# thygate/stable-diffusion-webui-depthmap-script

Measured on AMD Instinct MI355X. Metric: depth+stereo pairs/sec @1024x1024, higher is better.
Workload: dtype f16 (network) / f64 (stereo, normal map); 1 GPU; BASELINE config c3: MiDaS 3.1 DPT BEiT-L/16 512 forward (fp16, random-init weights seed 0, net 512x512, 1025 tokens) + depth->u16 + create_stereoimages(polylines_sharp, left-right, divergence 2.5%) + create_normalmap (Sobel 3) on 32 x 1024x1024 RGB per GPU, inputs resident in HBM; depth_network=dpt_beit_large_512, height=1024, width=1024, forward_launch=eager, library_convolutions=MIOpen, heuristic solver choice, overlap=single stream, parallelism=units sharded over 1 GPU(s), no data-path collective

## Files before the change

stable-diffusion-webui-depthmap-script_amd/csrc/ds_linear.hip:

```cpp
#include "ds_common.h"

#include <stdlib.h>
#include <atomic>
#include <type_traits>

typedef _Float16 lf16x8 __attribute__((ext_vector_type(8)));
typedef __bf16 lbf16x8 __attribute__((ext_vector_type(8)));
typedef _Float16 lf16x4 __attribute__((ext_vector_type(4)));
typedef __bf16 lbf16x4 __attribute__((ext_vector_type(4)));
typedef float lf32x16 __attribute__((ext_vector_type(16)));
typedef float lf32x4 __attribute__((ext_vector_type(4)));

#if defined(DS_EXPERIMENTS) && defined(DS_LIN_MFMA32)
#define LN_MF16 0
#else
#define LN_MF16 1
#endif

#define LN_THREADS 512
#define LN_LDS_BYTES 131072
#define LN_HALF 16384
#define LN_B_BASE 65536

template <int BF16> struct ln_traits;
template <> struct ln_traits<0> {
    typedef _Float16 T; typedef lf16x8 V8; typedef lf16x4 V4;
    static __device__ __forceinline__ lf32x16 mfma(V8 a, V8 b, lf32x16 c) { return __builtin_amdgcn_mfma_f32_32x32x16_f16(a, b, c, 0, 0, 0); }
    static __device__ __forceinline__ lf32x4 mfma16(V8 a, V8 b, lf32x4 c) { return __builtin_amdgcn_mfma_f32_16x16x32_f16(a, b, c, 0, 0, 0); }
    static __device__ __forceinline__ V8 relu(V8 v)
    {
        typedef unsigned lu32x4 __attribute__((ext_vector_type(4)));
        const lu32x4 x = __builtin_bit_cast(lu32x4, v);
        unsigned r0, r1, r2, r3;
        asm("v_pk_max_f16 %0, %1, 0" : "=v"(r0) : "v"(x[0]));
        asm("v_pk_max_f16 %0, %1, 0" : "=v"(r1) : "v"(x[1]));
        asm("v_pk_max_f16 %0, %1, 0" : "=v"(r2) : "v"(x[2]));
        asm("v_pk_max_f16 %0, %1, 0" : "=v"(r3) : "v"(x[3]));
        return __builtin_bit_cast(V8, (lu32x4){r0, r1, r2, r3});
    }
};
template <> struct ln_traits<1> {
    typedef __bf16 T; typedef lbf16x8 V8; typedef lbf16x4 V4;
    static __device__ __forceinline__ lf32x16 mfma(V8 a, V8 b, lf32x16 c) { return __builtin_amdgcn_mfma_f32_32x32x16_bf16(a, b, c, 0, 0, 0); }
    static __device__ __forceinline__ lf32x4 mfma16(V8 a, V8 b, lf32x4 c) { return __builtin_amdgcn_mfma_f32_16x16x32_bf16(a, b, c, 0, 0, 0); }
    static __device__ __forceinline__ V8 relu(V8 v)
    {
        typedef unsigned lu32x4 __attribute__((ext_vector_type(4)));
        lu32x4 x = __builtin_bit_cast(lu32x4, v);
#pragma unroll
        for (int i = 0; i < 4; ++i) {
            const unsigned neg = (x[i] >> 15) & 0x00010001u;
            x[i] &= ~(neg * 0xffffu);
        }
        return __builtin_bit_cast(V8, x);
    }
};

struct LinParams {
    const void *x, *w, *bias;
    const void *res1, *res2;
    const void *zeros;
    void *y;
    int M, N, K;
    int nbm, nbn;
    int bnw;
    int ablate;
    int stagger;
    int H, W, C, cpt, magic;
    long long ldy;
    const void *gamma;
    int early;
    int n_main;
    int vt_np, vt_c;
    unsigned vt_magic;
    int ps_w, ps_s, ps_c;
    unsigned ps_w_magic, ps_c_magic;
    int rd_np, rd_n, rd_dummy;
    unsigned rd_magic;
    float *rg_ws;
    int *rg_cnt;
    int rg_ksl;
    int th_nrb;
    int kt_kind;
    const float2 *ln_stats;
    const float *ln_colsum;
};

__device__ __forceinline__ void ln_tile_origin(const LinParams &P, const int tile, int &bm0, int &bn0)
{
    const int grp8 = tile / (8 * P.nbn), rem8 = tile - grp8 * (8 * P.nbn);
    const int rows8 = min(8, P.nbm - 8 * grp8);
    const int bn = rem8 / rows8, bm = 8 * grp8 + (rem8 - bn * rows8);
    bm0 = min(bm * 256, P.M - 256);
    bn0 = bn * P.bnw;
}

template <int VT>
__device__ __forceinline__ size_t ln_out_off(const LinParams &P, const int row, const int col)
{
    if (VT == 0) return (size_t)row * P.ldy + col;
    if (VT == 1) {
        const unsigned b = __umulhi((unsigned)col, P.vt_magic);
        const unsigned n = (unsigned)col - b * (unsigned)P.vt_np;
        return ((size_t)b * P.vt_c + row) * (size_t)P.vt_np + n;
    }
    if (VT == 2) {
        const unsigned q = __umulhi((unsigned)row, P.ps_w_magic), x = (unsigned)row - q * (unsigned)P.ps_w;
        const unsigned t = __umulhi((unsigned)col, P.ps_c_magic), co = (unsigned)col - t * (unsigned)P.ps_c;
        const unsigned ky = t / (unsigned)P.ps_s, kx = t - ky * (unsigned)P.ps_s;
        const size_t opix = ((size_t)q * P.ps_s + ky) * ((size_t)P.ps_w * P.ps_s) + (size_t)x * P.ps_s + kx;
        return opix * (size_t)P.ps_c + co;
    }
    const unsigned b = __umulhi((unsigned)row, P.rd_magic), t = (unsigned)row - b * (unsigned)P.rd_np;
    const bool live = t >= 1u && t < (unsigned)P.rd_n;
    const size_t orow = live ? (size_t)b * (size_t)(P.rd_n - 1) + (t - 1u) : (size_t)P.rd_dummy;
    return orow * (size_t)P.ldy + col;
}
template <int VT>
__device__ __forceinline__ size_t ln_res_off(const LinParams &P, const int row, const int col)
{
    if (VT != 3) return ln_out_off<VT>(P, row, col);
    const unsigned b = __umulhi((unsigned)row, P.rd_magic);
    return (size_t)b * (size_t)P.ldy + col;
}

__device__ __forceinline__ float ln_gelu(float v)
{
    const float u = fminf(fabsf(v), 6.0f);
    float q = 1.8896206483987044e-06f;
    q = __builtin_fmaf(q, u, -6.268127617659047e-05f);
    q = __builtin_fmaf(q, u, 0.000938866869546473f);
    q = __builtin_fmaf(q, u, -0.008539456874132156f);
    q = __builtin_fmaf(q, u, 0.054020676761865616f);
    q = __builtin_fmaf(q, u, 0.45840978622436523f);
    q = __builtin_fmaf(q, u, 1.1512691974639893f);
    q = __builtin_fmaf(q, u, 0.9999943375587463f);
    const float h = __builtin_amdgcn_exp2f(-q);
    return __builtin_fmaf(-u, h, fmaxf(v, 0.0f));
}
typedef float lf32x2 __attribute__((ext_vector_type(2)));
__device__ __forceinline__ lf32x2 ln_gelu2(lf32x2 v)
{
    const lf32x2 u = {fminf(fabsf(v[0]), 6.0f), fminf(fabsf(v[1]), 6.0f)};
    lf32x2 q = {1.8896206483987044e-06f, 1.8896206483987044e-06f};
#define LN_PK(c) q = __builtin_elementwise_fma(q, u, (lf32x2){c, c})
    LN_PK(-6.268127617659047e-05f); LN_PK(0.000938866869546473f); LN_PK(-0.008539456874132156f); LN_PK(0.054020676761865616f);
    LN_PK(0.45840978622436523f); LN_PK(1.1512691974639893f); LN_PK(0.9999943375587463f);
#undef LN_PK
    const lf32x2 h = {__builtin_amdgcn_exp2f(-q[0]), __builtin_amdgcn_exp2f(-q[1])};
    const lf32x2 r = {fmaxf(v[0], 0.0f), fmaxf(v[1], 0.0f)};
    return __builtin_elementwise_fma(-u, h, r);
}

__device__ __forceinline__ void ln_dma_s(const void *base_uniform, unsigned voff, unsigned lds_uniform)
{
    asm volatile("s_mov_b32 m0, %2\n\ts_nop 0\n\tglobal_load_lds_dwordx4 %0, %1" ::"v"(voff), "s"(base_uniform), "s"(lds_uniform) : "memory");
}
__device__ __forceinline__ void ln_dma_v(const void *ptr, unsigned lds_uniform)
{
    asm volatile("s_mov_b32 m0, %1\n\ts_nop 0\n\tglobal_load_lds_dwordx4 %0, off" ::"v"(ptr), "s"(lds_uniform) : "memory");
}

#ifdef DS_EXPERIMENTS
#define LN_ABLATE(bit) (P.ablate & (bit))
#define LN_STAGGER() (P.stagger)
#else
#define LN_ABLATE(bit) 0
#define LN_STAGGER() 0
#endif
#define LN_WAIT_VM(n) asm volatile("s_waitcnt vmcnt(" #n ")" ::: "memory")
template <int N> __device__ __forceinline__ void ln_wait_vm() { asm volatile("s_waitcnt vmcnt(%0)" ::"n"(N) : "memory"); }
#define LN_WAIT_LGKM0() asm volatile("s_waitcnt lgkmcnt(0)" ::: "memory")
#define LN_BARRIER()                              \
    do {                                          \
        __builtin_amdgcn_sched_barrier(0);        \
        __builtin_amdgcn_s_barrier();             \
        __builtin_amdgcn_sched_barrier(0);        \
    } while (0)

template <int BF16, int EPI, int CONV, int RES, int VT = 0, int NH = 0>
__global__ __launch_bounds__(LN_THREADS) void k_linear256(LinParams P)
{
    typedef ln_traits<BF16> TR;
    typedef typename TR::T T;
    typedef typename TR::V8 V8;
    extern __shared__ __attribute__((aligned(1024))) unsigned char lds[];

    const int tid = threadIdx.x;
    const int lane = tid & 63;
    const int wid = __builtin_amdgcn_readfirstlane(tid >> 6);
    const int wr = wid >> 2, wc = wid & 3;

    const int nwg = P.n_main;
    const int K = P.K;
    const int rowbytes = (CONV ? P.C : K) * (int)sizeof(T);

    unsigned srcA[2], srcB[2];
    int rowA[2];
#pragma unroll
    for (int i = 0; i < 2; ++i) {
        const int c = 2 * wid + i;
        const int j = 8 * c + (lane >> 3);
        const int slot = (lane & 7) ^ ((j >> 1) & 7);
        rowA[i] = (j >> 6) * 128 + (j & 63);
        srcA[i] = (unsigned)rowA[i] * (unsigned)rowbytes + slot * 16;
        const int col = NH ? j : (j >> 5) * 64 + (j & 31);
        srcB[i] = (unsigned)col * (unsigned)K * (unsigned)sizeof(T) + slot * 16;
    }
    const unsigned a_half = 64u * (unsigned)rowbytes;
    const unsigned b_half = NH ? 0u : 32u * (unsigned)K * (unsigned)sizeof(T);
    const unsigned lds_stage = (unsigned)(size_t)(__attribute__((address_space(3))) void *)lds + (unsigned)(2 * wid) * 1024u;

    int bm0 = 0, bn0 = 0;
    const unsigned char *xb = nullptr, *wb = nullptr;
    unsigned okA = 0;
    auto set_tile = [&](const int orig) {
        const int xcd = orig & 7, q8 = nwg >> 3, r8 = nwg & 7;
        const int tile = (xcd < r8 ? xcd * (q8 + 1) : r8 * (q8 + 1) + (xcd - r8) * q8) + (orig >> 3);
        ln_tile_origin(P, tile, bm0, bn0);
        xb = (const unsigned char *)P.x + (size_t)bm0 * rowbytes;
        wb = (const unsigned char *)P.w + (size_t)bn0 * K * sizeof(T);
        if (CONV) {
            okA = 0;
#pragma unroll
            for (int i = 0; i < 2; ++i)
#pragma unroll
                for (int h = 0; h < 2; ++h) {
                    const unsigned pix = (unsigned)(bm0 + rowA[i] + 64 * h) % (unsigned)(P.H * P.W);
                    const int py = (int)(pix / (unsigned)P.W), px = (int)(pix % (unsigned)P.W);
                    const unsigned bits = (py > 0 ? 1u : 0u) | 2u | (py < P.H - 1 ? 4u : 0u) | (px > 0 ? 8u : 0u) | 16u | (px < P.W - 1 ? 32u : 0u);
                    okA |= bits << (6 * (2 * h + i));
                }
        }
    };

#define LN_STAGE(kind, kt, s)                                                                                            \
    do {                                                                                                                 \
        unsigned koff_ = (unsigned)(kt) * 128u;                                                                          \
        const unsigned dst_ = ((kind) >> 1) * LN_B_BASE + ((kind) & 1) * 2 * LN_HALF + (s) * LN_HALF + lds_stage;   \
        int dy_ = 0, dx_ = 0, aoff_ = (int)koff_;                                                                        \
        if (CONV) {               \
            const int cc_ = ((kt) * 7282) >> 16, tap_ = (kt) - 9 * cc_;       \
            dy_ = ((tap_ * 11) >> 5) - 1; dx_ = tap_ - 3 * (dy_ + 1) - 1;                                                \
            aoff_ = cc_ * 128 + (dy_ * P.W + dx_) * rowbytes;                                                            \
            koff_ = (unsigned)(tap_ * P.cpt + cc_) * 128u;                            \
        }                                                                                                                \
                   \
        const unsigned char *ub_ = ((kind) < 2) ? xb + ((long)aoff_ + (long)(((kind) & 1) * a_half))                     \
                                                : wb + (size_t)(((kind) & 1) * b_half + koff_);                          \
        _Pragma("unroll") for (int i_ = 0; i_ < 2; ++i_) {                                                               \
            if (CONV && (kind) < 2) {                                                                                    \
                const unsigned sh_ = 6 * (2 * ((kind) & 1) + i_);                                                        \
                const unsigned ok_ = (okA >> (sh_ + dy_ + 1)) & (okA >> (sh_ + 4 + dx_)) & 1u;                           \
                const unsigned char *g_ = ok_ ? ub_ + (size_t)srcA[i_] : (const unsigned char *)P.zeros;                 \
                ln_dma_v(g_, dst_ + i_ * 1024);                                                                          \
            } else {                                                                                                     \
                ln_dma_s(ub_, ((kind) < 2) ? srcA[i_] : srcB[i_], dst_ + i_ * 1024);                                     \
            }                                                                                                            \
        }                                                                                                                \
    } while (0)

    constexpr bool MF16 = LN_MF16 && CONV == 0;
    constexpr int NKS = MF16 ? 2 : 4;
    unsigned offA[NKS], offB[NKS];
#pragma unroll
    for (int ks = 0; ks < NKS; ++ks) {
        const int lrow = MF16 ? (lane & 15) : (lane & 31);
        const unsigned sl = (unsigned)((MF16 ? 4 * ks + (lane >> 4) : 2 * ks + (lane >> 5)) ^ ((lane >> 1) & 7)) << 4;
        offA[ks] = (unsigned)(wr * 64 + lrow) * 128u + sl;
        offB[ks] = LN_B_BASE + (unsigned)(wc * 32 + lrow) * 128u + sl;
    }
    const int c8 = MF16 ? 16 * ((lane >> 4) & 1) + 8 * (lane >> 5) : 8 * (lane >> 5);
    constexpr int NBK = MF16 ? 1 : 2;
    constexpr int NBIAS = 2 * NBK;
    V8 bv[2][2];
#define LN_LOAD_BIAS()                                                                                                   \
    do {                                                                                                                 \
        const T *bias_ = (const T *)P.bias;                                                                              \
        _Pragma("unroll") for (int hb_ = 0; hb_ < 2; ++hb_) _Pragma("unroll") for (int k_ = 0; k_ < NBK; ++k_) {         \
            const int c_ = bn0 + (NH ? wc * 32 : wc * 64 + hb_ * 32) + c8 + 16 * k_;                                     \
            bv[hb_][k_] = *(const V8 *)(bias_ ? bias_ + c_ : (const T *)P.w);                                            \
        }                                                                                                                \
    } while (0)
#define LN_ZERO_NULL_BIAS()                                                                                              \
    do {                                                                                                                 \
        if (!P.bias) {                                                                                                   \
            _Pragma("unroll") for (int hb_ = 0; hb_ < 2; ++hb_) _Pragma("unroll") for (int k_ = 0; k_ < NBK; ++k_)       \
                _Pragma("unroll") for (int t_ = 0; t_ < 8; ++t_) bv[hb_][k_][t_] = (T)0.f;                               \
        }                                                                                                                \
    } while (0)
    V8 fa[2][2][4];
    V8 fb[2][4];
    lf32x16 acc[2][2][2];
    V8 fa16[2][4][2];
    V8 fb16[2][2][2];
    lf32x4 acc16[2][4][2][2];

#define LN_READ_A(h, s)                                                                                                  \
    do {                                                                                                                 \
        if constexpr (MF16) {                                                                                            \
            _Pragma("unroll") for (int rb_ = 0; rb_ < 4; ++rb_) _Pragma("unroll") for (int ks_ = 0; ks_ < 2; ++ks_)      \
                fa16[h][rb_][ks_] = *(const V8 *)(lds + offA[ks_] + ((h) * 2 * LN_HALF + (s) * LN_HALF + rb_ * 2048));   \
        } else {                                                                                                         \
            _Pragma("unroll") for (int rb_ = 0; rb_ < 2; ++rb_) _Pragma("unroll") for (int ks_ = 0; ks_ < 4; ++ks_)      \
                fa[h][rb_][ks_] = *(const V8 *)(lds + offA[ks_] + ((h) * 2 * LN_HALF + (s) * LN_HALF + rb_ * 4096));     \
        }                                                                                                                \
    } while (0)
#define LN_RELU_A(h)                                                                                                     \
    do {                                                                                                                 \
        if constexpr (CONV == 2) {                                                                                       \
            _Pragma("unroll") for (int rb_ = 0; rb_ < 2; ++rb_) _Pragma("unroll") for (int ks_ = 0; ks_ < 4; ++ks_)      \
                fa[h][rb_][ks_] = TR::relu(fa[h][rb_][ks_]);                                                             \
        }                                                                                                                \
    } while (0)
#define LN_READ_B(h, s)                                                                                                  \
    do {                                                                                                                 \
        if constexpr (MF16) {                                                                                            \
            _Pragma("unroll") for (int cb_ = 0; cb_ < 2; ++cb_) _Pragma("unroll") for (int ks_ = 0; ks_ < 2; ++ks_)      \
                if (!(NH && (h) == 1)) fb16[h][cb_][ks_] = *(const V8 *)(lds + offB[ks_] + ((h) * 2 * LN_HALF + (s) * LN_HALF + cb_ * 2048)); \
        } else {                                                                                                         \
            _Pragma("unroll") for (int ks_ = 0; ks_ < 4; ++ks_)                                                          \
                if (!(NH && (h) == 1)) fb[h][ks_] = *(const V8 *)(lds + offB[ks_] + ((h) * 2 * LN_HALF + (s) * LN_HALF)); \
        }                                                                                                                \
    } while (0)
#define LN_MMA_PART(ha, hb)                                                                                              \
    do {                                                                                                                 \
        if (!(NH && (hb) == 1)) {                                                                                        \
            if constexpr (MF16) {                                                                                        \
                _Pragma("unroll") for (int ks_ = 0; ks_ < 2; ++ks_) _Pragma("unroll") for (int rb_ = 0; rb_ < 4; ++rb_)  \
                    _Pragma("unroll") for (int cb_ = 0; cb_ < 2; ++cb_)                                                  \
                        acc16[ha][rb_][hb][cb_] = TR::mfma16(fb16[hb][cb_][ks_], fa16[ha][rb_][ks_], acc16[ha][rb_][hb][cb_]); \
            } else {                                                                                                     \
                _Pragma("unroll") for (int ks_ = 0; ks_ < 4; ++ks_) _Pragma("unroll") for (int rb_ = 0; rb_ < 2; ++rb_)  \
                    acc[ha][rb_][hb] = TR::mfma(fb[hb][ks_], fa[ha][rb_][ks_], acc[ha][rb_][hb]);                        \
            }                                                                                                            \
        }                                                                                                                \
    } while (0)

    const int nt = K >> 6, ni = nt >> 1;

#define LN_PROLOGUE()                                                                                                    \
    do {                                                                                                                 \
        LN_STAGE(0, 0, 0); LN_STAGE(2, 0, 0); LN_STAGE(3, 0, 0); LN_STAGE(1, 0, 0);                                      \
        LN_STAGE(0, 1, 1); LN_STAGE(2, 1, 1); LN_STAGE(3, 1, 1);                                                         \
    } while (0)

#define LN_PHASE_END(ha, hb)                                                                                             \
    do {                                                                                                                 \
        LN_BARRIER(); LN_WAIT_LGKM0();                                                                                   \
        __builtin_amdgcn_s_setprio(1);                                                                                   \
        LN_MMA_PART(ha, hb);                                                                                             \
        __builtin_amdgcn_s_setprio(0);                                                                                   \
        LN_BARRIER();                                                                                                    \
    } while (0)
#define LN_MEM(READ, STAGE)                                                                                              \
    do { READ; STAGE; } while (0)

    auto iteration = [&](const int i, auto kind_c) {
        constexpr int KIND = decltype(kind_c)::value;
        constexpr bool LAST = KIND == 1;
        const int e2 = 2 * i + 2, o2 = 2 * i + 3;
#define LN_WAIT_HEAD()                                                                                                   \
        do {                                                                                                             \
            if constexpr (KIND == 2) { if constexpr (NH) LN_WAIT_VM(18); else LN_WAIT_VM(26); }                          \
            else if constexpr (KIND == 1) ln_wait_vm<10 + NBIAS>();                                                   \
            else LN_WAIT_VM(10);                                                                                         \
        } while (0)
        LN_MEM(LN_READ_B(0, 0), LN_STAGE(1, 2 * i + 1, 1)); LN_WAIT_HEAD();
        LN_PHASE_END(0, 0);
        if constexpr (!LAST) { LN_MEM(LN_READ_B(1, 0), LN_STAGE(0, e2, 0)); LN_WAIT_HEAD(); } else { LN_READ_B(1, 0); ln_wait_vm<8 + NBIAS>(); }
        LN_PHASE_END(0, 1);
        if constexpr (!LAST) { LN_MEM(LN_READ_A(1, 0), LN_STAGE(2, e2, 0)); LN_RELU_A(1); LN_WAIT_HEAD(); } else { LN_READ_A(1, 0); LN_RELU_A(1); ln_wait_vm<6 + NBIAS>(); }
        LN_PHASE_END(1, 1);
        if constexpr (!LAST) { LN_MEM(LN_READ_A(0, 1), LN_STAGE(3, e2, 0)); LN_RELU_A(0); LN_WAIT_HEAD(); } else { LN_READ_A(0, 1); LN_RELU_A(0); ln_wait_vm<4 + NBIAS>(); }
        LN_PHASE_END(1, 0);
        if constexpr (!LAST) { LN_MEM(LN_READ_B(0, 1), LN_STAGE(1, e2, 0)); LN_WAIT_HEAD(); } else { LN_READ_B(0, 1); ln_wait_vm<2 + NBIAS>(); }
        LN_PHASE_END(0, 0);
#undef LN_WAIT_HEAD
        if constexpr (!LAST) { LN_MEM(LN_READ_B(1, 1), LN_STAGE(0, o2, 1)); LN_WAIT_VM(10); } else { LN_READ_B(1, 1); LN_WAIT_VM(0); }
        LN_PHASE_END(0, 1);
        if constexpr (!LAST) { LN_MEM(LN_READ_A(1, 1), LN_STAGE(2, o2, 1)); LN_RELU_A(1); LN_WAIT_VM(10); } else { LN_READ_A(1, 1); LN_RELU_A(1); }
        LN_PHASE_END(1, 1);
        if constexpr (!LAST) { LN_MEM(LN_READ_A(0, 0), LN_STAGE(3, o2, 1)); LN_RELU_A(0); LN_WAIT_VM(10); }
        LN_PHASE_END(1, 0);
    };
    if (LN_STAGGER() > 0 && ((blockIdx.x >> 3) & 1)) {
        const unsigned long long t0 = wall_clock64();
        while (wall_clock64() - t0 < (unsigned long long)LN_STAGGER()) __builtin_amdgcn_s_sleep(32);
    }
    const bool early = P.early != 0;
    bool stores_ahead = false;
    set_tile(blockIdx.x);
    LN_PROLOGUE();
    for (int orig = blockIdx.x;;) {
    if constexpr (MF16) {
#pragma unroll
        for (int a = 0; a < 2; ++a)
#pragma unroll
            for (int b = 0; b < 4; ++b)
#pragma unroll
                for (int c = 0; c < 2; ++c)
#pragma unroll
                    for (int d = 0; d < 2; ++d)
#pragma unroll
                        for (int r = 0; r < 4; ++r) acc16[a][b][c][d][r] = 0.f;
    } else {
#pragma unroll
        for (int a = 0; a < 2; ++a)
#pragma unroll
            for (int b = 0; b < 2; ++b)
#pragma unroll
                for (int c = 0; c < 2; ++c)
#pragma unroll
                    for (int r = 0; r < 16; ++r) acc[a][b][c][r] = 0.f;
    }
    if (!early) LN_WAIT_VM(10);
    else if (stores_ahead) { if constexpr (NH) LN_WAIT_VM(18); else LN_WAIT_VM(26); }
    else LN_WAIT_VM(0);
    LN_BARRIER();
    LN_READ_A(0, 0);
    LN_WAIT_LGKM0();
    LN_RELU_A(0);
    if (wr == 1) LN_BARRIER();
    if (LN_ABLATE(2)) {
        LN_LOAD_BIAS();
        LN_WAIT_VM(0);
        if (wr == 0) LN_BARRIER();
    } else {
        int i0 = 0;
        if (early && ni >= 2) { iteration(0, std::integral_constant<int, 2>()); i0 = 1; }
        for (int i = i0; i < ni - 1; ++i) iteration(i, std::integral_constant<int, 0>());
        LN_LOAD_BIAS();
        iteration(ni - 1, std::integral_constant<int, 1>());
        if (wr == 0) LN_BARRIER();
    }
    const int cbm0 = bm0, cbn0 = bn0;
    const int next = orig + (int)gridDim.x;
    const int hi8 = 8 * (lane >> 5);
    LN_ZERO_NULL_BIAS();
    T *yb = (T *)P.y;
    const T *r1 = (const T *)P.res1, *r2 = (const T *)P.res2;
    if (early && next < nwg) {
#pragma unroll
        for (int hb = 0; hb < 2; ++hb)
#pragma unroll
            for (int k = 0; k < NBK; ++k) {
                asm volatile("" ::"v"(bv[hb][k]));
            }
        set_tile(next);
        LN_PROLOGUE();
    }

    if constexpr (MF16) {
        V8 gv[2];
        if (EPI == 3) {
#pragma unroll
            for (int hb = 0; hb < 2; ++hb) gv[hb] = *(const V8 *)((const T *)P.gamma + cbn0 + (NH ? wc * 32 : wc * 64 + hb * 32) + c8);
        }
        constexpr int NHB = NH ? 1 : 2;
        const int wcol = NH ? wc * 32 : wc * 64;
#pragma unroll
        for (int ha = 0; ha < 2; ++ha)
#pragma unroll
            for (int rb = 0; rb < 4; ++rb) {
                const int row = cbm0 + wr * 128 + ha * 64 + rb * 16 + (lane & 15);
                const int col = cbn0 + wcol + c8;
                const size_t o0 = (size_t)row * P.ldy + col;
                V8 ra[2], rb2[2];
                constexpr bool LNF = EPI == 4 || EPI == 5;
                float2 st_row = {1.f, 0.f};
                float cs_row = 0.f;
                static_assert(!LNF || VT == 0 || VT == 1, "the folded LayerNorm exists for the row-major and the V^T store only");
                if (LNF && VT == 0) st_row = P.ln_stats[row];
                if (LNF && VT == 1) cs_row = P.ln_colsum[row];
#pragma unroll
                for (int hb = 0; hb < NHB; ++hb) {
                    if (RES >= 1) ra[hb] = *(const V8 *)(r1 + (VT == 3 ? ln_res_off<VT>(P, row, col + hb * 32) : o0 + hb * 32));
                    if (RES >= 2) rb2[hb] = *(const V8 *)(r2 + o0 + hb * 32);
                }
#pragma unroll
                for (int hb = 0; hb < NHB; ++hb) {
                    float v[8];
#pragma unroll
                    for (int t = 0; t < 4; ++t) {
                        const float fa = acc16[ha][rb][hb][0][t], fb = acc16[ha][rb][hb][1][t];
                        const auto sw = __builtin_amdgcn_permlane16_swap(__float_as_uint(fa), __float_as_uint(fb), false, false);
                        v[t] = __uint_as_float(sw[0]);
                        v[4 + t] = __uint_as_float(sw[1]);
                    }
                    V8 o;
                    if (LNF) {
                        const int c0 = col + hb * 32;
                        if (!VT) {
                            const float4 s0 = *(const float4 *)(P.ln_colsum + c0), s1 = *(const float4 *)(P.ln_colsum + c0 + 4);
                            const float sc[8] = {s0.x, s0.y, s0.z, s0.w, s1.x, s1.y, s1.z, s1.w};
#pragma unroll
                            for (int t = 0; t < 8; ++t) v[t] = __builtin_fmaf(v[t], st_row.x, st_row.y * sc[t]);
                        } else {
                            const float4 *sp = (const float4 *)(P.ln_stats + c0);
                            const float4 q0 = sp[0], q1 = sp[1], q2 = sp[2], q3 = sp[3];
                            const float rs[8] = {q0.x, q0.z, q1.x, q1.z, q2.x, q2.z, q3.x, q3.z};
                            const float nm[8] = {q0.y, q0.w, q1.y, q1.w, q2.y, q2.w, q3.y, q3.w};
#pragma unroll
                            for (int t = 0; t < 8; ++t) v[t] = __builtin_fmaf(v[t], rs[t], nm[t] * cs_row);
                        }
                    }
#pragma unroll
                    for (int t = 0; t < 8; t += 2) {
                        lf32x2 u = {v[t] + (float)bv[hb][0][t], v[t + 1] + (float)bv[hb][0][t + 1]};
                        if (EPI == 3) u *= (lf32x2){(float)gv[hb][t], (float)gv[hb][t + 1]};
                        if (RES >= 1) u += (lf32x2){(float)ra[hb][t], (float)ra[hb][t + 1]};
                        if (RES >= 2) u += (lf32x2){(float)rb2[hb][t], (float)rb2[hb][t + 1]};
                        if (EPI == 1 || EPI == 5) u = ln_gelu2(u);
                        if (EPI == 2) u = (lf32x2){fmaxf(u[0], 0.f), fmaxf(u[1], 0.f)};
                        o[t] = (T)u[0];
                        o[t + 1] = (T)u[1];
                    }
                    T *dst = yb + (VT ? ln_out_off<VT>(P, row, col + hb * 32) : o0 + hb * 32);
                    if (!LN_ABLATE(1)) *(V8 *)dst = o;
                    else asm volatile("" ::"v"(o));
                }
            }
    } else {
        V8 gv[2][2];
        if (EPI == 3) {
#pragma unroll
            for (int hb = 0; hb < 2; ++hb)
#pragma unroll
                for (int k = 0; k < 2; ++k) gv[hb][k] = *(const V8 *)((const T *)P.gamma + cbn0 + (NH ? wc * 32 : wc * 64 + hb * 32) + hi8 + 16 * k);
        }
        constexpr int NHB = NH ? 1 : 2;
        const int wcol = NH ? wc * 32 : wc * 64;
#pragma unroll
        for (int ha = 0; ha < 2; ++ha)
#pragma unroll
            for (int rb = 0; rb < 2; ++rb) {
                const int rl = ha * 64 + rb * 32 + (lane & 31);
                const size_t o0 = (size_t)(cbm0 + wr * 128 + rl) * P.ldy + cbn0 + wcol + hi8;
                auto out_off = [&](const int hb_, const int k_) -> size_t {
                    return VT ? ln_out_off<VT>(P, cbm0 + wr * 128 + rl, cbn0 + wcol + hi8 + hb_ * 32 + 16 * k_) : o0 + hb_ * 32 + 16 * k_;
                };
                V8 ra[2][2], rb2[2][2];
                constexpr bool LNF = EPI == 4 || EPI == 5;
                float2 st_row = {1.f, 0.f};
                float cs_row = 0.f;
                static_assert(!LNF || VT == 0 || VT == 1, "the folded LayerNorm exists for the row-major and the V^T store only");
                if (LNF && VT == 0) st_row = P.ln_stats[cbm0 + wr * 128 + rl];
                if (LNF && VT == 1) cs_row = P.ln_colsum[cbm0 + wr * 128 + rl];
#pragma unroll
                for (int hb = 0; hb < NHB; ++hb)
#pragma unroll
                    for (int k = 0; k < 2; ++k) {
                        if (RES >= 1) ra[hb][k] = *(const V8 *)(r1 + (VT == 3 ? ln_res_off<VT>(P, cbm0 + wr * 128 + rl, cbn0 + wcol + hi8 + hb * 32 + 16 * k) : o0 + hb * 32 + 16 * k));
                        if (RES >= 2) rb2[hb][k] = *(const V8 *)(r2 + o0 + hb * 32 + 16 * k);
                    }
#pragma unroll
                for (int hb = 0; hb < NHB; ++hb)
#pragma unroll
                    for (int k = 0; k < 2; ++k) {
                        float v[8];
#pragma unroll
                        for (int t = 0; t < 4; ++t) {
                            const float fa = acc[ha][rb][hb][8 * k + t], fb = acc[ha][rb][hb][8 * k + 4 + t];
                            const auto sw = __builtin_amdgcn_permlane32_swap(__float_as_uint(fa), __float_as_uint(fb), false, false);
                            v[t] = __uint_as_float(sw[0]);
                            v[4 + t] = __uint_as_float(sw[1]);
                        }
                        V8 o;
                        if (LNF) {
                            const int c0 = cbn0 + wcol + hi8 + hb * 32 + 16 * k;
                            if (!VT) {
                                const float4 s0 = *(const float4 *)(P.ln_colsum + c0), s1 = *(const float4 *)(P.ln_colsum + c0 + 4);
                                const float sc[8] = {s0.x, s0.y, s0.z, s0.w, s1.x, s1.y, s1.z, s1.w};
#pragma unroll
                                for (int t = 0; t < 8; ++t) v[t] = __builtin_fmaf(v[t], st_row.x, st_row.y * sc[t]);
                            } else {
                                const float4 *sp = (const float4 *)(P.ln_stats + c0);
                                const float4 q0 = sp[0], q1 = sp[1], q2 = sp[2], q3 = sp[3];
                                const float rs[8] = {q0.x, q0.z, q1.x, q1.z, q2.x, q2.z, q3.x, q3.z};
                                const float nm[8] = {q0.y, q0.w, q1.y, q1.w, q2.y, q2.w, q3.y, q3.w};
#pragma unroll
                                for (int t = 0; t < 8; ++t) v[t] = __builtin_fmaf(v[t], rs[t], nm[t] * cs_row);
                            }
                        }
#pragma unroll
// ... 524 lines not shown
    }
    P.n_main = ntiles - ragged;
    const int deep = O.ragged_ring ? O.ragged_ring == 6 : 8 * ragged <= grid;
    bool thin = false;
    int th_nrb = 0;
    if constexpr (CONV == 0 && VT == 0 && RES <= 1) {
        th_nrb = (P.M - (P.nbm - 1) * 256 + 31) / 32;
        thin = O.ragged_thin && ragged > 0 && ragged == P.nbn && P.nbm >= 2 && (P.nbm - 1) % 8 == 0 && P.K % 128 == 0 && P.N % 64 == 0 &&
               O.ragged_ksplit <= 1 && th_nrb * (P.N / 64) <= ctx->ncu;
    }
    P.th_nrb = th_nrb;
    int ksl = 0;
    if (CONV == 0 && ragged && !thin && deep && 8 * ragged * (int)sizeof(int) <= LN_RG_COUNTER_BYTES && ln_ksplit_arch_ok(ctx)) {
        const int nt = P.K / 64;
        while (nt >= O.ragged_ksplit_min && (2 << ksl) <= O.ragged_ksplit && 8 * ragged * (2 << ksl) <= grid && nt % (2 << ksl) == 0 &&
               nt / (2 << ksl) >= O.ragged_ksplit_keep) ++ksl;
    }
    if (ksl > 0) {
        const int rc = ln_ragged_workspace(ctx, grid, stream);
        if (rc == DS_OK) { P.rg_cnt = (int *)ctx->lin_ws; P.rg_ws = (float *)((char *)ctx->lin_ws + LN_RG_COUNTER_BYTES); }
        else if (rc == 1) ksl = 0;
        else return rc;
    }
    P.rg_ksl = ksl;
    const int kt0 = ds_kt_begin(ctx, P.kt_kind, stream);
    hipLaunchKernelGGL(fn, dim3(P.n_main < grid ? P.n_main : grid), dim3(LN_THREADS), LN_LDS_BYTES, stream, P);
    ds_kt_end(ctx, P.kt_kind, kt0, stream);
    if constexpr (CONV == 0) {
        const int kt1 = ragged ? ds_kt_begin(ctx, P.kt_kind + DS_KT_RAGGED, stream) : -1;
        if (thin) {
            if constexpr (VT == 0 && RES <= 1) hipLaunchKernelGGL((k_linear_thin<BF16, EPI, RES>), dim3(th_nrb * (P.N / 64)), dim3(LN_THREADS), 6 * RG_SLOT, stream, P);
        } else if (ragged && deep && O.ragged_pipe) hipLaunchKernelGGL((k_linear_ragged<BF16, EPI, RES, VT, 6, 1>), dim3((8 * ragged) << ksl), dim3(LN_THREADS), 6 * RG_SLOT, stream, P);
        else if (ragged && deep) hipLaunchKernelGGL((k_linear_ragged<BF16, EPI, RES, VT, 6>), dim3((8 * ragged) << ksl), dim3(LN_THREADS), 6 * RG_SLOT, stream, P);
        else if (ragged) hipLaunchKernelGGL((k_linear_ragged<BF16, EPI, RES, VT, 3>), dim3(8 * ragged), dim3(LN_THREADS), 3 * RG_SLOT, stream, P);
        ds_kt_end(ctx, P.kt_kind + DS_KT_RAGGED, kt1, stream);
    }
    DS_HIP_CHECK(hipGetLastError());
    return DS_OK;
}

template <int BF16>
static int ln_dispatch_dense(ds_ctx *ctx, const LinParams &P, int act, hipStream_t st)
{
    if (act == 1) return ln_launch<BF16, 1, 0, 0>(ctx, P, st);
    if (act == 2) return ln_launch<BF16, 2, 0, 0>(ctx, P, st);
    return ln_launch<BF16, 0, 0, 0>(ctx, P, st);
}

template <int BF16>
static int ln_dispatch_conv(ds_ctx *ctx, const LinParams &P, int act, hipStream_t st)
{
    const int res = P.res1 ? (P.res2 ? 2 : 1) : 0;
    if (act & 4) {
        if (P.N % 256 == 0 && (act & 3) == 2 && res == 0) return ln_launch<BF16, 2, 2, 0>(ctx, P, st);
        ds_set_error("ds_conv3x3_nhwc: act 4 (ReLU on x) is built for act 2 | 4 without residual operands and out_channels %% 256 == 0");
        return DS_EUNSUPPORTED;
    }
    if (P.N % 256 != 0) {
        if (act == 2) return ln_launch<BF16, 2, 1, 0, 0, 1>(ctx, P, st);
        return ln_launch<BF16, 0, 1, 0, 0, 1>(ctx, P, st);
    }
    if (act == 2) {
        if (res == 2) return ln_launch<BF16, 2, 1, 2>(ctx, P, st);
        if (res == 1) return ln_launch<BF16, 2, 1, 1>(ctx, P, st);
        return ln_launch<BF16, 2, 1, 0>(ctx, P, st);
    }
    if (res == 2) return ln_launch<BF16, 0, 1, 2>(ctx, P, st);
    if (res == 1) return ln_launch<BF16, 0, 1, 1>(ctx, P, st);
    return ln_launch<BF16, 0, 1, 0>(ctx, P, st);
}

DS_API int ds_linear(ds_ctx *ctx, const void *x, const void *w, const void *bias, void *y, int64_t rows, int64_t out_features,
                     int64_t in_features, int64_t ldy, int act, int dtype, void *stream)
{
    DS_REQUIRE(ctx && x && w && y, DS_EINVAL, "ds_linear: null argument");
    DS_REQUIRE(rows >= 256 && rows < (1ll << 31) - 256, DS_EINVAL, "ds_linear: rows must be >= 256 (one tile)");
    DS_REQUIRE(out_features > 0 && out_features % 256 == 0, DS_EINVAL, "ds_linear: out_features must be a multiple of 256");
    DS_REQUIRE(in_features >= 128 && in_features % 128 == 0 && in_features <= 16384, DS_EINVAL,
               "ds_linear: in_features must be a multiple of 128 (<= 16384)");
    DS_REQUIRE(ldy >= out_features && ldy % 8 == 0, DS_EINVAL, "ds_linear: ldy must be >= out_features and a multiple of 8");
    DS_REQUIRE(((uintptr_t)x & 15) == 0 && ((uintptr_t)w & 15) == 0 && ((uintptr_t)y & 15) == 0 && (!bias || ((uintptr_t)bias & 15) == 0), DS_EINVAL,
               "ds_linear: x, w (the LDS-DMA sources), y and bias must be 16-byte aligned");
    DS_REQUIRE(act >= 0 && act <= 2, DS_EINVAL, "ds_linear: act must be 0 (none), 1 (erf-GELU) or 2 (ReLU)");
    DS_REQUIRE(dtype == DS_DTYPE_F16 || dtype == DS_DTYPE_BF16, DS_EINVAL, "ds_linear: dtype must be f16 or bf16");
    LinParams P;
    memset(&P, 0, sizeof(P));
    P.x = x; P.w = w; P.bias = bias; P.y = y;
    P.M = (int)rows; P.N = (int)out_features; P.K = (int)in_features;
    P.nbm = (int)((rows + 255) / 256); P.nbn = (int)(out_features / 256);
    P.ldy = ldy;
    P.kt_kind = act == 1 ? DS_KT_LINEAR_GELU : DS_KT_LINEAR;
#ifdef DS_EXPERIMENTS
    P.ablate = getenv("DS_LIN_ABLATE") ? atoi(getenv("DS_LIN_ABLATE")) : 0;
    P.stagger = getenv("DS_LIN_STAGGER_US") ? (int)(atof(getenv("DS_LIN_STAGGER_US")) * 100.0) : 0;
#endif
    return dtype == DS_DTYPE_F16 ? ln_dispatch_dense<0>(ctx, P, act, (hipStream_t)stream) : ln_dispatch_dense<1>(ctx, P, act, (hipStream_t)stream);
}

DS_API int ds_linear_residual(ds_ctx *ctx, const void *x, const void *w, const void *bias, const void *gamma, const void *res, void *y,
                              int64_t rows, int64_t out_features, int64_t in_features, int dtype, void *stream)
{
    DS_REQUIRE(ctx && x && w && y && res, DS_EINVAL, "ds_linear_residual: null argument");
    DS_REQUIRE(rows >= 256 && rows < (1ll << 31) - 256, DS_EINVAL, "ds_linear_residual: rows must be >= 256 (one tile)");
    DS_REQUIRE(out_features > 0 && out_features % 256 == 0, DS_EINVAL, "ds_linear_residual: out_features must be a multiple of 256");
    DS_REQUIRE(in_features >= 128 && in_features % 128 == 0 && in_features <= 16384, DS_EINVAL,
               "ds_linear_residual: in_features must be a multiple of 128 (<= 16384)");
    DS_REQUIRE(dtype == DS_DTYPE_F16 || dtype == DS_DTYPE_BF16, DS_EINVAL, "ds_linear_residual: dtype must be f16 or bf16");
    DS_REQUIRE(((uintptr_t)x & 15) == 0 && ((uintptr_t)w & 15) == 0 && ((uintptr_t)y & 15) == 0 && ((uintptr_t)res & 15) == 0 &&
               ((uintptr_t)bias & 15) == 0 && ((uintptr_t)gamma & 15) == 0 && y != res,
               DS_EINVAL, "ds_linear_residual: x, w, y, res, bias and gamma must be 16-byte aligned, and y must not alias res");
    LinParams P;
    memset(&P, 0, sizeof(P));
    P.x = x; P.w = w; P.bias = bias; P.gamma = gamma; P.res1 = res; P.y = y;
    P.M = (int)rows; P.N = (int)out_features; P.K = (int)in_features;
    P.nbm = (int)((rows + 255) / 256); P.nbn = (int)(out_features / 256);
    P.ldy = out_features;
    P.kt_kind = DS_KT_LINEAR_RESIDUAL;
    hipStream_t st = (hipStream_t)stream;
    if (dtype == DS_DTYPE_F16) return gamma ? ln_launch<0, 3, 0, 1>(ctx, P, st) : ln_launch<0, 0, 0, 1>(ctx, P, st);
    return gamma ? ln_launch<1, 3, 0, 1>(ctx, P, st) : ln_launch<1, 0, 0, 1>(ctx, P, st);
}

DS_API int ds_conv3x3_nhwc(ds_ctx *ctx, const void *x, const void *w, const void *bias, const void *res1, const void *res2, void *y,
                           int batch, int height, int width, int in_channels, int out_channels, int act, int dtype, void *stream)
{
    DS_REQUIRE(ctx && x && w && y, DS_EINVAL, "ds_conv3x3_nhwc: null argument");
    DS_REQUIRE(batch > 0 && height > 0 && width > 0 && height < 32768 && width < 32768, DS_EINVAL, "ds_conv3x3_nhwc: bad image shape");
    DS_REQUIRE((int64_t)batch * height * width < (1ll << 31) - 256 && (int64_t)batch * height * width >= 256, DS_EINVAL,
               "ds_conv3x3_nhwc: batch * height * width must be in [256, 2^31)");
    DS_REQUIRE(in_channels >= 64 && in_channels % 64 == 0 && (9 * in_channels / 64) % 2 == 0 && in_channels <= 4096, DS_EINVAL,
               "ds_conv3x3_nhwc: in_channels must be a multiple of 128 (<= 4096)");
    DS_REQUIRE(out_channels > 0 && out_channels % 128 == 0, DS_EINVAL, "ds_conv3x3_nhwc: out_channels must be a multiple of 128");
    DS_REQUIRE(out_channels % 256 == 0 || (!res1 && !res2), DS_EUNSUPPORTED,
               "ds_conv3x3_nhwc: residual operands need out_channels to be a multiple of 256 (the 128-column tiles have no residual epilogue)");
    DS_REQUIRE(act == 0 || act == 2 || act == 6, DS_EINVAL, "ds_conv3x3_nhwc: act must be 0 (none), 2 (ReLU) or 6 (ReLU, and ReLU on x)");
    DS_REQUIRE(dtype == DS_DTYPE_F16 || dtype == DS_DTYPE_BF16, DS_EINVAL, "ds_conv3x3_nhwc: dtype must be f16 or bf16");
    DS_REQUIRE(((uintptr_t)x & 15) == 0 && ((uintptr_t)w & 15) == 0 && ((uintptr_t)y & 15) == 0 && (!bias || ((uintptr_t)bias & 15) == 0) &&
               ((uintptr_t)res1 & 15) == 0 && ((uintptr_t)res2 & 15) == 0,
               DS_EINVAL, "ds_conv3x3_nhwc: x, w, y, bias, res1 and res2 must be 16-byte aligned");
    int rc = ds_ctx_reserve(ctx, &ctx->zero_line, &ctx->zero_line_bytes, 256);
    if (rc != DS_OK) return rc;
    if (!ctx->zero_line_cleared) {
        DS_HIP_CHECK(hipMemsetAsync(ctx->zero_line, 0, 256, (hipStream_t)stream));
        DS_HIP_CHECK(hipStreamSynchronize((hipStream_t)stream));
        ctx->zero_line_cleared = 1;
    }
    LinParams P;
    memset(&P, 0, sizeof(P));
    if (!res1 && res2) { res1 = res2; res2 = nullptr; }
    P.x = x; P.w = w; P.bias = bias; P.res1 = res1; P.res2 = res2; P.y = y; P.zeros = ctx->zero_line;
    P.M = batch * height * width; P.N = out_channels; P.K = 9 * in_channels;
    P.nbm = (P.M + 255) / 256; P.nbn = out_channels % 256 == 0 ? out_channels / 256 : out_channels / 128;
    P.H = height; P.W = width; P.C = in_channels; P.cpt = in_channels / 64; P.magic = 65536 / P.cpt + 1;
    for (int kt = 0; kt < P.K / 64; ++kt)
        DS_REQUIRE(((kt * 7282) >> 16) == kt / 9, DS_EUNSUPPORTED, "ds_conv3x3_nhwc: K-tile arithmetic does not cover %d channels", in_channels);
    P.ldy = out_channels;
    P.kt_kind = DS_KT_CONV3X3;
#ifdef DS_EXPERIMENTS
    P.ablate = getenv("DS_LIN_ABLATE") ? atoi(getenv("DS_LIN_ABLATE")) : 0;
    P.stagger = getenv("DS_LIN_STAGGER_US") ? (int)(atof(getenv("DS_LIN_STAGGER_US")) * 100.0) : 0;
#endif
    return dtype == DS_DTYPE_F16 ? ln_dispatch_conv<0>(ctx, P, act, (hipStream_t)stream) : ln_dispatch_conv<1>(ctx, P, act, (hipStream_t)stream);
}

DS_API int ds_linear_vt(ds_ctx *ctx, const void *w_v, const void *h, void *vt, int64_t channels, int64_t batch, int64_t tokens,
                        int64_t in_features, int dtype, void *stream)
{
    DS_REQUIRE(ctx && w_v && h && vt, DS_EINVAL, "ds_linear_vt: null argument");
    DS_REQUIRE(channels >= 256, DS_EINVAL, "ds_linear_vt: channels must be >= 256 (one tile)");
    DS_REQUIRE(batch > 0 && tokens > 0 && tokens % 8 == 0 && (batch * tokens) % 256 == 0 && batch * tokens < (1ll << 31) - 256, DS_EINVAL,
               "ds_linear_vt: tokens must be a multiple of 8 and batch * tokens a multiple of 256");
    DS_REQUIRE(batch * tokens * tokens < (1ll << 32), DS_EUNSUPPORTED, "ds_linear_vt: batch * tokens^2 must stay below 2^32");
    DS_REQUIRE(in_features >= 128 && in_features % 128 == 0 && in_features <= 16384, DS_EINVAL,
               "ds_linear_vt: in_features must be a multiple of 128 (<= 16384)");
    DS_REQUIRE(dtype == DS_DTYPE_F16 || dtype == DS_DTYPE_BF16, DS_EINVAL, "ds_linear_vt: dtype must be f16 or bf16");
    DS_REQUIRE(((uintptr_t)w_v & 15) == 0 && ((uintptr_t)h & 15) == 0 && ((uintptr_t)vt & 15) == 0, DS_EINVAL,
               "ds_linear_vt: w_v, h and vt must be 16-byte aligned");
    LinParams P;
    memset(&P, 0, sizeof(P));
    P.x = w_v; P.w = h; P.y = vt;
    P.M = (int)channels; P.N = (int)(batch * tokens); P.K = (int)in_features;
    P.nbm = (int)((channels + 255) / 256); P.nbn = (int)(batch * tokens / 256);
    P.ldy = batch * tokens;
    P.vt_np = (int)tokens; P.vt_c = (int)channels; P.vt_magic = (unsigned)((1ull << 32) / (unsigned long long)tokens + 1ull);
    P.kt_kind = DS_KT_LINEAR_VT;
    hipStream_t st = (hipStream_t)stream;
    return dtype == DS_DTYPE_F16 ? ln_launch<0, 0, 0, 0, 1>(ctx, P, st) : ln_launch<1, 0, 0, 0, 1>(ctx, P, st);
}

DS_API int ds_linear_shuffle(ds_ctx *ctx, const void *x, const void *w, const void *bias, void *y, int64_t pixels, int64_t in_features,
                             int width, int stride, int out_channels, int dtype, void *stream)
{
    DS_REQUIRE(ctx && x && w && y, DS_EINVAL, "ds_linear_shuffle: null argument");
    DS_REQUIRE(stride >= 1 && stride <= 8 && width >= 1 && out_channels >= 8 && out_channels % 8 == 0, DS_EINVAL,
               "ds_linear_shuffle: stride must be 1..8, out_channels a multiple of 8");
    const int64_t n = (int64_t)stride * stride * out_channels;
    DS_REQUIRE(pixels >= 256 && pixels % width == 0 && pixels < (1ll << 31) - 256, DS_EINVAL,
               "ds_linear_shuffle: pixels must be >= 256 (one tile) and a whole number of image rows");
    DS_REQUIRE(n % 256 == 0, DS_EUNSUPPORTED, "ds_linear_shuffle: stride^2 * out_channels must be a multiple of 256 (got %lld)", (long long)n);
    DS_REQUIRE(in_features >= 128 && in_features % 128 == 0 && in_features <= 16384, DS_EINVAL,
               "ds_linear_shuffle: in_features must be a multiple of 128 (<= 16384)");
    DS_REQUIRE(pixels * width < (1ll << 32) && n * out_channels < (1ll << 32) && pixels * n < (1ll << 40), DS_EUNSUPPORTED,
               "ds_linear_shuffle: shape too large for the index arithmetic");
    DS_REQUIRE(dtype == DS_DTYPE_F16 || dtype == DS_DTYPE_BF16, DS_EINVAL, "ds_linear_shuffle: dtype must be f16 or bf16");
    DS_REQUIRE(((uintptr_t)x & 15) == 0 && ((uintptr_t)w & 15) == 0 && ((uintptr_t)y & 15) == 0 && (!bias || ((uintptr_t)bias & 15) == 0), DS_EINVAL,
               "ds_linear_shuffle: x, w, y and bias must be 16-byte aligned");
    LinParams P;
    memset(&P, 0, sizeof(P));
    P.x = x; P.w = w; P.bias = bias; P.y = y;
    P.M = (int)pixels; P.N = (int)n; P.K = (int)in_features;
    P.nbm = (int)((pixels + 255) / 256); P.nbn = (int)(n / 256);
    P.ldy = n;
    P.ps_w = width; P.ps_s = stride; P.ps_c = out_channels;
    P.ps_w_magic = (unsigned)((1ull << 32) / (unsigned long long)width + 1ull);
    P.ps_c_magic = (unsigned)((1ull << 32) / (unsigned long long)out_channels + 1ull);
    P.kt_kind = DS_KT_LINEAR_SHUFFLE;
    hipStream_t st = (hipStream_t)stream;
    return dtype == DS_DTYPE_F16 ? ln_launch<0, 0, 0, 0, 2>(ctx, P, st) : ln_launch<1, 0, 0, 0, 2>(ctx, P, st);
}

DS_API int ds_linear_readout(ds_ctx *ctx, const void *x, const void *w_tok, const void *cls_vec, void *y, int64_t images,
                             int64_t tokens_padded, int64_t tokens, int64_t out_features, int64_t in_features, int dtype, void *stream)
{
    DS_REQUIRE(ctx && x && w_tok && cls_vec && y, DS_EINVAL, "ds_linear_readout: null argument");
    DS_REQUIRE(images > 0 && tokens >= 2 && tokens <= tokens_padded, DS_EINVAL, "ds_linear_readout: need 2 <= tokens <= tokens_padded");
    const int64_t rows = images * tokens_padded;
    DS_REQUIRE(rows >= 256 && rows < (1ll << 31) - 256 && rows * tokens_padded < (1ll << 32), DS_EINVAL,
               "ds_linear_readout: images * tokens_padded must be in [256, 2^31) and images * tokens_padded^2 below 2^32");
    DS_REQUIRE(out_features > 0 && out_features % 256 == 0, DS_EINVAL, "ds_linear_readout: out_features must be a multiple of 256");
    DS_REQUIRE(in_features >= 128 && in_features % 128 == 0 && in_features <= 16384, DS_EINVAL,
               "ds_linear_readout: in_features must be a multiple of 128 (<= 16384)");
    DS_REQUIRE(dtype == DS_DTYPE_F16 || dtype == DS_DTYPE_BF16, DS_EINVAL, "ds_linear_readout: dtype must be f16 or bf16");
    DS_REQUIRE(((uintptr_t)x & 15) == 0 && ((uintptr_t)w_tok & 15) == 0 && ((uintptr_t)y & 15) == 0 && ((uintptr_t)cls_vec & 15) == 0, DS_EINVAL,
               "ds_linear_readout: x, w_tok, cls_vec and y must be 16-byte aligned");
    LinParams P;
    memset(&P, 0, sizeof(P));
    P.x = x; P.w = w_tok; P.res1 = cls_vec; P.y = y;
    P.M = (int)rows; P.N = (int)out_features; P.K = (int)in_features;
    P.nbm = (int)((rows + 255) / 256); P.nbn = (int)(out_features / 256);
    P.ldy = out_features;
    P.rd_np = (int)tokens_padded; P.rd_n = (int)tokens; P.rd_dummy = (int)(images * (tokens - 1));
    P.rd_magic = (unsigned)((1ull << 32) / (unsigned long long)tokens_padded + 1ull);
    P.kt_kind = DS_KT_LINEAR_READOUT;
    hipStream_t st = (hipStream_t)stream;
    return dtype == DS_DTYPE_F16 ? ln_launch<0, 1, 0, 1, 3>(ctx, P, st) : ln_launch<1, 1, 0, 1, 3>(ctx, P, st);
}

DS_API int ds_linear_ln(ds_ctx *ctx, const void *x, const void *w_scaled, const float *colsum, const void *bias, const void *stats, void *y,
                        int64_t rows, int64_t out_features, int64_t in_features, int64_t ldy, int act, int dtype, void *stream)
{
    DS_REQUIRE(ctx && x && w_scaled && colsum && stats && y, DS_EINVAL, "ds_linear_ln: null argument");
    DS_REQUIRE(rows >= 256 && rows < (1ll << 31) - 256, DS_EINVAL, "ds_linear_ln: rows must be >= 256 (one tile)");
    DS_REQUIRE(out_features > 0 && out_features % 256 == 0, DS_EINVAL, "ds_linear_ln: out_features must be a multiple of 256");
    DS_REQUIRE(in_features >= 128 && in_features % 128 == 0 && in_features <= 16384, DS_EINVAL, "ds_linear_ln: in_features must be a multiple of 128 (<= 16384)");
    DS_REQUIRE(ldy >= out_features && ldy % 8 == 0, DS_EINVAL, "ds_linear_ln: ldy must be >= out_features and a multiple of 8");
    DS_REQUIRE(((uintptr_t)x & 15) == 0 && ((uintptr_t)w_scaled & 15) == 0 && ((uintptr_t)y & 15) == 0 && (!bias || ((uintptr_t)bias & 15) == 0) &&
               ((uintptr_t)colsum & 15) == 0 && ((uintptr_t)stats & 15) == 0, DS_EINVAL, "ds_linear_ln: operands must be 16-byte aligned");
    DS_REQUIRE(act == 0 || act == 1, DS_EINVAL, "ds_linear_ln: act must be 0 (none) or 1 (erf-GELU)");
    DS_REQUIRE(dtype == DS_DTYPE_F16 || dtype == DS_DTYPE_BF16, DS_EINVAL, "ds_linear_ln: dtype must be f16 or bf16");
    LinParams P;
    memset(&P, 0, sizeof(P));
    P.x = x; P.w = w_scaled; P.bias = bias; P.y = y; P.ln_stats = (const float2 *)stats; P.ln_colsum = colsum;
    P.M = (int)rows; P.N = (int)out_features; P.K = (int)in_features;
    P.nbm = (int)((rows + 255) / 256); P.nbn = (int)(out_features / 256);
    P.ldy = ldy;
    P.kt_kind = act == 1 ? DS_KT_LINEAR_GELU : DS_KT_LINEAR;
    hipStream_t st = (hipStream_t)stream;
    if (dtype == DS_DTYPE_F16) return act == 1 ? ln_launch<0, 5, 0, 0>(ctx, P, st) : ln_launch<0, 4, 0, 0>(ctx, P, st);
    return act == 1 ? ln_launch<1, 5, 0, 0>(ctx, P, st) : ln_launch<1, 4, 0, 0>(ctx, P, st);
}

DS_API int ds_linear_vt_ln(ds_ctx *ctx, const void *w_v_scaled, const float *colsum, const void *x, const void *stats, void *vt,
                           int64_t channels, int64_t batch, int64_t tokens, int64_t in_features, int dtype, void *stream)
{
    DS_REQUIRE(ctx && w_v_scaled && colsum && x && stats && vt, DS_EINVAL, "ds_linear_vt_ln: null argument");
    DS_REQUIRE(channels >= 256, DS_EINVAL, "ds_linear_vt_ln: channels must be >= 256 (one tile)");
    DS_REQUIRE(batch > 0 && tokens > 0 && tokens % 8 == 0 && (batch * tokens) % 256 == 0 && batch * tokens < (1ll << 31) - 256, DS_EINVAL,
               "ds_linear_vt_ln: tokens must be a multiple of 8 and batch * tokens a multiple of 256");
    DS_REQUIRE(batch * tokens * tokens < (1ll << 32), DS_EUNSUPPORTED, "ds_linear_vt_ln: batch * tokens^2 must stay below 2^32");
    DS_REQUIRE(in_features >= 128 && in_features % 128 == 0 && in_features <= 16384, DS_EINVAL, "ds_linear_vt_ln: in_features must be a multiple of 128 (<= 16384)");
    DS_REQUIRE(dtype == DS_DTYPE_F16 || dtype == DS_DTYPE_BF16, DS_EINVAL, "ds_linear_vt_ln: dtype must be f16 or bf16");
    DS_REQUIRE(((uintptr_t)w_v_scaled & 15) == 0 && ((uintptr_t)x & 15) == 0 && ((uintptr_t)vt & 15) == 0 && ((uintptr_t)colsum & 15) == 0 &&
               ((uintptr_t)stats & 15) == 0, DS_EINVAL, "ds_linear_vt_ln: operands must be 16-byte aligned");
    LinParams P;
    memset(&P, 0, sizeof(P));
    P.x = w_v_scaled; P.w = x; P.y = vt; P.ln_stats = (const float2 *)stats; P.ln_colsum = colsum;
    P.M = (int)channels; P.N = (int)(batch * tokens); P.K = (int)in_features;
    P.nbm = (int)((channels + 255) / 256); P.nbn = (int)(batch * tokens / 256);
    P.ldy = batch * tokens;
    P.vt_np = (int)tokens; P.vt_c = (int)channels; P.vt_magic = (unsigned)((1ull << 32) / (unsigned long long)tokens + 1ull);
    P.kt_kind = DS_KT_LINEAR_VT;
    hipStream_t st = (hipStream_t)stream;
    return dtype == DS_DTYPE_F16 ? ln_launch<0, 4, 0, 0, 1>(ctx, P, st) : ln_launch<1, 4, 0, 0, 1>(ctx, P, st);
}
```

Baseline: 888.5 pairs/s.

## Use 16x16x32 MFMA path for conv3x3 kernels with late bias load

Switches the conv3x3 (CONV=1) GEMM path from 32x32x16 MFMA to 16x16x32 MFMA fragments, deriving the second k-slice LDS offset with an XOR to save registers, and deferring the bias load to the last iteration to reduce register pressure. Also replaces integer division/modulo in the per-tile boundary mask computation with magic-number reciprocal divmod. The ReLU-prologue conv variant (CONV=2) keeps the old path unless an experiment flag is set. The aim is better MFMA throughput and fewer registers in the DPT refinement convolutions, with some risk of extra LDS reads or a worse schedule.

```diff
diff --git a/stable-diffusion-webui-depthmap-script_amd/csrc/ds_linear.hip b/stable-diffusion-webui-depthmap-script_amd/csrc/ds_linear.hip
--- a/stable-diffusion-webui-depthmap-script_amd/csrc/ds_linear.hip
+++ b/stable-diffusion-webui-depthmap-script_amd/csrc/ds_linear.hip
@@ -15,6 +15,11 @@
 #define LN_MF16 0
 #else
 #define LN_MF16 1
+#endif
+#if defined(DS_EXPERIMENTS) && defined(DS_LIN_CONV2_MFMA16)
+#define LN_MF16_CONV2 1
+#else
+#define LN_MF16_CONV2 0
 #endif
 
 #define LN_THREADS 512
@@ -84,7 +89,17 @@
     int kt_kind;
     const float2 *ln_stats;
     const float *ln_colsum;
+    unsigned hw_magic, w_magic;
 };
+
+__device__ __forceinline__ unsigned ln_divmod(const unsigned n, const unsigned d, const unsigned magic, unsigned &rem)
+{
+    unsigned q = __umulhi(n, magic);
+    unsigned r = n - q * d;
+    if (r >= d) { r -= d; ++q; }
+    rem = r;
+    return q;
+}
 
 __device__ __forceinline__ void ln_tile_origin(const LinParams &P, const int tile, int &bm0, int &bn0)
 {
@@ -226,8 +241,9 @@
             for (int i = 0; i < 2; ++i)
 #pragma unroll
                 for (int h = 0; h < 2; ++h) {
-                    const unsigned pix = (unsigned)(bm0 + rowA[i] + 64 * h) % (unsigned)(P.H * P.W);
-                    const int py = (int)(pix / (unsigned)P.W), px = (int)(pix % (unsigned)P.W);
+                    unsigned pix, upx;
+                    ln_divmod((unsigned)(bm0 + rowA[i] + 64 * h), (unsigned)(P.H * P.W), P.hw_magic, pix);
+                    const int py = (int)ln_divmod(pix, (unsigned)P.W, P.w_magic, upx), px = (int)upx;
                     const unsigned bits = (py > 0 ? 1u : 0u) | 2u | (py < P.H - 1 ? 4u : 0u) | (px > 0 ? 8u : 0u) | 16u | (px < P.W - 1 ? 32u : 0u);
                     okA |= bits << (6 * (2 * h + i));
                 }
@@ -260,9 +276,9 @@
         }                                                                                                                \
     } while (0)
 
-    constexpr bool MF16 = LN_MF16 && CONV == 0;
-    constexpr int NKS = MF16 ? 2 : 4;
-    unsigned offA[NKS], offB[NKS];
+    constexpr bool MF16 = LN_MF16 && (CONV != 2 || LN_MF16_CONV2);
+    constexpr int NKS = MF16 ? (CONV ? 1 : 2) : 4;
+    unsigned offA[4], offB[4];
 #pragma unroll
     for (int ks = 0; ks < NKS; ++ks) {
         const int lrow = MF16 ? (lane & 15) : (lane & 31);
@@ -272,7 +288,8 @@
     }
     const int c8 = MF16 ? 16 * ((lane >> 4) & 1) + 8 * (lane >> 5) : 8 * (lane >> 5);
     constexpr int NBK = MF16 ? 1 : 2;
-    constexpr int NBIAS = 2 * NBK;
+    constexpr bool LATE_BIAS = MF16 && CONV != 0;
+    constexpr int NBIAS = LATE_BIAS ? 0 : 2 * NBK;
     V8 bv[2][2];
 #define LN_LOAD_BIAS()                                                                                                   \
     do {                                                                                                                 \
@@ -296,11 +313,13 @@
     V8 fb16[2][2][2];
     lf32x4 acc16[2][4][2][2];
 
+#define LN_OFF1(off) ({ unsigned o1_; if constexpr (CONV != 0) asm volatile("v_xor_b32 %0, 64, %1" : "=v"(o1_) : "v"(off[0])); else o1_ = off[1]; o1_; })
 #define LN_READ_A(h, s)                                                                                                  \
     do {                                                                                                                 \
         if constexpr (MF16) {                                                                                            \
+            const unsigned o_[2] = {offA[0], LN_OFF1(offA)};                                                              \
             _Pragma("unroll") for (int rb_ = 0; rb_ < 4; ++rb_) _Pragma("unroll") for (int ks_ = 0; ks_ < 2; ++ks_)      \
-                fa16[h][rb_][ks_] = *(const V8 *)(lds + offA[ks_] + ((h) * 2 * LN_HALF + (s) * LN_HALF + rb_ * 2048));   \
+                fa16[h][rb_][ks_] = *(const V8 *)(lds + o_[ks_] + ((h) * 2 * LN_HALF + (s) * LN_HALF + rb_ * 2048));     \
         } else {                                                                                                         \
             _Pragma("unroll") for (int rb_ = 0; rb_ < 2; ++rb_) _Pragma("unroll") for (int ks_ = 0; ks_ < 4; ++ks_)      \
                 fa[h][rb_][ks_] = *(const V8 *)(lds + offA[ks_] + ((h) * 2 * LN_HALF + (s) * LN_HALF + rb_ * 4096));     \
@@ -308,7 +327,10 @@
     } while (0)
 #define LN_RELU_A(h)                                                                                                     \
     do {                                                                                                                 \
-        if constexpr (CONV == 2) {                                                                                       \
+        if constexpr (CONV == 2 && MF16) {                                                                               \
+            _Pragma("unroll") for (int rb_ = 0; rb_ < 4; ++rb_) _Pragma("unroll") for (int ks_ = 0; ks_ < 2; ++ks_)      \
+                fa16[h][rb_][ks_] = TR::relu(fa16[h][rb_][ks_]);                                                         \
+        } else if constexpr (CONV == 2) {                                                                                \
             _Pragma("unroll") for (int rb_ = 0; rb_ < 2; ++rb_) _Pragma("unroll") for (int ks_ = 0; ks_ < 4; ++ks_)      \
                 fa[h][rb_][ks_] = TR::relu(fa[h][rb_][ks_]);                                                             \
         }                                                                                                                \
@@ -316,8 +338,11 @@
 #define LN_READ_B(h, s)                                                                                                  \
     do {                                                                                                                 \
         if constexpr (MF16) {                                                                                            \
-            _Pragma("unroll") for (int cb_ = 0; cb_ < 2; ++cb_) _Pragma("unroll") for (int ks_ = 0; ks_ < 2; ++ks_)      \
-                if (!(NH && (h) == 1)) fb16[h][cb_][ks_] = *(const V8 *)(lds + offB[ks_] + ((h) * 2 * LN_HALF + (s) * LN_HALF + cb_ * 2048)); \
+            if (!(NH && (h) == 1)) {                                                                                     \
+                const unsigned o_[2] = {offB[0], LN_OFF1(offB)};                                                          \
+                _Pragma("unroll") for (int cb_ = 0; cb_ < 2; ++cb_) _Pragma("unroll") for (int ks_ = 0; ks_ < 2; ++ks_)  \
+                    fb16[h][cb_][ks_] = *(const V8 *)(lds + o_[ks_] + ((h) * 2 * LN_HALF + (s) * LN_HALF + cb_ * 2048)); \
+            }                                                                                                            \
         } else {                                                                                                         \
             _Pragma("unroll") for (int ks_ = 0; ks_ < 4; ++ks_)                                                          \
                 if (!(NH && (h) == 1)) fb[h][ks_] = *(const V8 *)(lds + offB[ks_] + ((h) * 2 * LN_HALF + (s) * LN_HALF)); \
@@ -379,7 +404,8 @@
 #undef LN_WAIT_HEAD
         if constexpr (!LAST) { LN_MEM(LN_READ_B(1, 1), LN_STAGE(0, o2, 1)); LN_WAIT_VM(10); } else { LN_READ_B(1, 1); LN_WAIT_VM(0); }
         LN_PHASE_END(0, 1);
-        if constexpr (!LAST) { LN_MEM(LN_READ_A(1, 1), LN_STAGE(2, o2, 1)); LN_RELU_A(1); LN_WAIT_VM(10); } else { LN_READ_A(1, 1); LN_RELU_A(1); }
+        if constexpr (!LAST) { LN_MEM(LN_READ_A(1, 1), LN_STAGE(2, o2, 1)); LN_RELU_A(1); LN_WAIT_VM(10); }
+        else { LN_READ_A(1, 1); if constexpr (LATE_BIAS) LN_LOAD_BIAS(); LN_RELU_A(1); }
         LN_PHASE_END(1, 1);
         if constexpr (!LAST) { LN_MEM(LN_READ_A(0, 0), LN_STAGE(3, o2, 1)); LN_RELU_A(0); LN_WAIT_VM(10); }
         LN_PHASE_END(1, 0);
@@ -404,6 +430,16 @@
                     for (int d = 0; d < 2; ++d)
 #pragma unroll
                         for (int r = 0; r < 4; ++r) acc16[a][b][c][d][r] = 0.f;
+        if constexpr (CONV != 0) {
+#pragma unroll
+            for (int a = 0; a < 2; ++a)
+#pragma unroll
+                for (int b = 0; b < 4; ++b)
+#pragma unroll
+                    for (int c = 0; c < 2; ++c)
+#pragma unroll
+                        for (int d = 0; d < 2; ++d) asm volatile("" : "+v"(acc16[a][b][c][d]));
+        }
     } else {
 #pragma unroll
         for (int a = 0; a < 2; ++a)
@@ -430,7 +466,7 @@
         int i0 = 0;
         if (early && ni >= 2) { iteration(0, std::integral_constant<int, 2>()); i0 = 1; }
         for (int i = i0; i < ni - 1; ++i) iteration(i, std::integral_constant<int, 0>());
-        LN_LOAD_BIAS();
+        if constexpr (!LATE_BIAS) LN_LOAD_BIAS();
         iteration(ni - 1, std::integral_constant<int, 1>());
         if (wr == 0) LN_BARRIER();
     }
@@ -1261,6 +1297,8 @@
     P.M = batch * height * width; P.N = out_channels; P.K = 9 * in_channels;
     P.nbm = (P.M + 255) / 256; P.nbn = out_channels % 256 == 0 ? out_channels / 256 : out_channels / 128;
     P.H = height; P.W = width; P.C = in_channels; P.cpt = in_channels / 64; P.magic = 65536 / P.cpt + 1;
+    const auto magic32 = [](const uint64_t d) { const uint64_t m = (1ull << 32) / d; return (unsigned)(m > 0xffffffffull ? 0xffffffffull : m); };
+    P.hw_magic = magic32((uint64_t)height * width); P.w_magic = magic32((uint64_t)width);
     for (int kt = 0; kt < P.K / 64; ++kt)
         DS_REQUIRE(((kt * 7282) >> 16) == kt / 9, DS_EUNSUPPORTED, "ds_conv3x3_nhwc: K-tile arithmetic does not cover %d channels", in_channels);
     P.ldy = out_channels;
```

Result: no change. 893.9 pairs/s, median of 6 (+0.6%).
